# meyer-lab/cmtf-pls

Measured on AMD Instinct MI355X. Metric: nipals_iters_per_sec, higher is better.
Workload: dtype f32

## Files before the change

### cmtf_pls_amd/_lib.py

```python
from __future__ import annotations

import ctypes
import os
from ctypes import c_char_p, c_double, c_int, c_int64, c_size_t, c_uint32, c_uint64, c_void_p

_HERE = os.path.dirname(os.path.abspath(__file__))
LIB_PATH = os.environ.get("CMTFPLS_LIB") or os.path.join(_HERE, "lib", "libcmtfpls.so")

_P = c_void_p

class XcovBlock(ctypes.Structure):
    _fields_ = [("S", _P), ("S2", _P), ("colcnt", _P), ("n_samples", c_double), ("order", c_int), ("A", c_int), ("B", c_int),
                ("n_squarings", c_int), ("Z", _P), ("wA", _P), ("wB", _P), ("info", _P)]


class KfoldState(ctypes.Structure):
    _fields_ = [("I", c_int), ("A", c_int), ("B", c_int), ("M", c_int), ("K", c_int), ("R", c_int)] + [
        (name, _P) for name in ("fold_of", "S", "mean", "Yk", "Gy", "WA", "WB", "Q", "Wa", "Wb", "T", "Gt", "coef", "Rm", "tm",
                                "Tout", "vec", "n_iter", "status", "part")]


class CvCoupledBlock(ctypes.Structure):
    _fields_ = [("X", _P), ("order", c_int), ("A", c_int), ("B", c_int)]

# ... 23 lines not shown
    "cmtfpls_rank1_workspace_bytes": (c_size_t, [c_int, c_int]),
    "cmtfpls_rank1_score_f64": (c_int, [_P, c_int, c_int, _P, _P, _P, c_int, _P, c_int, _P, _P, c_size_t, _P]),
    "cmtfpls_rank1_f64": (c_int, [_P, c_int, c_int, _P, _P, _P, _P, c_int, _P, c_size_t, _P]),
    "cmtfpls_rank1_launches_f64": (c_int, [_P, c_int, c_int, _P, _P, _P, _P, c_int, _P, c_size_t, _P]),
    "cmtfpls_rank1_chain_enable": (None, [c_int]),
    "cmtfpls_rank1_chain_enabled": (c_int, []),
    "cmtfpls_normalize_f64": (c_int, [_P, c_int64, _P, _P]),
    "cmtfpls_rank1_tensor_workspace_bytes": (c_size_t, [_P, c_int]),
    "cmtfpls_rank1_tensor_f64": (c_int, [_P, _P, c_int, c_double, _P, c_int, _P, c_int, _P, c_size_t, _P]),
    "cmtfpls_kron_f64": (c_int, [_P, c_int, _P, c_int, _P, _P]),
    "cmtfpls_xcov_workspace_bytes": (c_size_t, [c_int64, c_int64, c_int]),
    "cmtfpls_xcov_f32": (c_int, [_P, c_int64, c_int64, _P, c_int, c_int, _P, c_int, _P, c_size_t, _P]),
    "cmtfpls_xcov_f64": (c_int, [_P, c_int64, c_int64, _P, c_int, c_int, _P, c_int, _P, c_size_t, _P]),
    "cmtfpls_quadform_f64": (c_int, [_P, c_int, _P, _P, _P, _P]),
    "cmtfpls_xcov_iterate_f64": (c_int, [_P, c_int, c_int, c_int, _P, _P, _P, _P, _P, c_int, _P, _P, _P, c_int, _P, c_size_t, _P, c_size_t, _P]),
    "cmtfpls_s_downdate_f64": (c_int, [_P, c_int, c_int, c_int, _P, _P, _P, _P, _P, _P]),
    "cmtfpls_project_rows_f32": (c_int, [_P, c_int64, c_int, c_int, c_int, _P, _P, _P, _P, c_int, _P]),
    "cmtfpls_project_rows_f64": (c_int, [_P, c_int64, c_int, c_int, c_int, _P, _P, _P, _P, c_int, _P]),
    "cmtfpls_project_rows2_f32": (c_int, [_P, c_int, c_int, _P, _P, _P, _P, c_int, c_int, _P, _P, _P, c_int64, c_int, _P, c_int, _P]),
    "cmtfpls_project_rows2_f64": (c_int, [_P, c_int, c_int, _P, _P, _P, _P, c_int, c_int, _P, _P, _P, c_int64, c_int, _P, c_int, _P]),
    "cmtfpls_project_rows_idx_f32": (c_int, [_P, _P, c_int64, c_int, c_int, c_int, _P, _P, _P, _P, c_int, _P]),
    "cmtfpls_project_rows_idx_f64": (c_int, [_P, _P, c_int64, c_int, c_int, c_int, _P, _P, _P, _P, c_int, _P]),
    "cmtfpls_project_rows2_idx_f32": (c_int, [_P, c_int, c_int, _P, _P, _P, _P, c_int, c_int, _P, _P, _P, _P, c_int64, c_int, _P, c_int, _P]),
    "cmtfpls_project_rows2_idx_f64": (c_int, [_P, c_int, c_int, _P, _P, _P, _P, c_int, c_int, _P, _P, _P, _P, c_int64, c_int, _P, c_int, _P]),
    "cmtfpls_allreduce_sum_f64": (c_int, [_P, _P, c_size_t, _P]),
    "cmtfpls_allreduce_sum_f32": (c_int, [_P, _P, c_size_t, _P]),
    "cmtfpls_axpy_scalar_f64": (c_int, [_P, c_int64, _P, _P, _P]),
    "cmtfpls_xcov_deflate_f32": (c_int, [_P, c_int64, c_int, c_int, _P, c_int, c_int, _P, _P, _P, _P, _P, _P, c_size_t, _P]),
    "cmtfpls_xcov_deflate_f64": (c_int, [_P, c_int64, c_int, c_int, _P, c_int, c_int, _P, _P, _P, _P, _P, _P, c_size_t, _P]),
    "cmtfpls_xcov_stats_workspace_bytes": (c_size_t, [c_int64, c_int64, c_int]),
# ... 170 lines not shown
```

### cmtf_pls_amd/backend.py

```python
from __future__ import annotations

import ctypes
from typing import Optional, Tuple

import torch

from . import _lib

_SUFFIX = {torch.float32: "f32", torch.float64: "f64"}


def _ptr(t: Optional[torch.Tensor]):
    return None if t is None else t.data_ptr()


def _int_pairs(pairs):
    flat = [int(v) for p in pairs for v in p]
    return (ctypes.c_int * len(flat))(*flat)


def chunk_size(n: int, per: int, budget: int, cap: Optional[int] = None) -> int:
    chunk = max(1, min(int(n), int(budget) // max(int(per), 1)))
    return chunk if cap is None else min(chunk, int(cap))

# ... 235 lines not shown
                          wB: torch.Tensor, status: torch.Tensor, q_new: torch.Tensor, G: torch.Tensor):
        M, P = S.shape
        wc = self._workspace("contract", self.lib.cmtfpls_mode0_contract_workspace_bytes(M, P))
        wr = self._workspace("rank1", self.lib.cmtfpls_rank1_workspace_bytes(A, B))
        keep = (S, q_cur, Z, wA, wB, status, q_new, G, wc, wr)
        fn = self.lib.cmtfpls_xcov_iterate_f64
        head = (_ptr(S), M, A, B, _ptr(q_cur), _ptr(Z), _ptr(wA), _ptr(wB), status[1:3].data_ptr())
        tail = (_ptr(wc), wc.numel(), _ptr(wr), wr.numel())
        qn, Gp, du2 = _ptr(q_new), _ptr(G), status[0:1].data_ptr()
        stream = self._stream

        def enqueue(n_squarings: int, first: bool, _keep=keep) -> None:
            rc = fn(*head, n_squarings, qn, Gp, du2, 1 if first else 0, *tail, stream())
            if rc:
                _lib.check(rc, "xcov_iterate")
        return enqueue

    def xcov_iterate(self, S: torch.Tensor, A: int, B: int, q_cur: torch.Tensor, Z: torch.Tensor, wA: torch.Tensor,
                     wB: torch.Tensor, info: torch.Tensor, n_squarings: int, q_new: torch.Tensor, G: torch.Tensor,
                     du2: torch.Tensor, first: bool) -> None:
        M, P = S.shape
        wc = self._workspace("contract", self.lib.cmtfpls_mode0_contract_workspace_bytes(M, P))
        wr = self._workspace("rank1", self.lib.cmtfpls_rank1_workspace_bytes(A, B))
        _lib.check(self.lib.cmtfpls_xcov_iterate_f64(_ptr(S), M, A, B, _ptr(q_cur), _ptr(Z), _ptr(wA), _ptr(wB), _ptr(info),
                                                     int(n_squarings), _ptr(q_new), _ptr(G), _ptr(du2), int(first),
                                                     _ptr(wc), wc.numel(), _ptr(wr), wr.numel(), self._stream()), "xcov_iterate")

    def xcov_blocks_plan(self, blocks, M: int, q_cur: torch.Tensor, tq: torch.Tensor, q_new: torch.Tensor, G: torch.Tensor,
                         status: torch.Tensor):
        nb = len(blocks)
# ... 785 lines not shown
```

### cmtf_pls_amd/csrc/rank1.hip

```cpp
#include "common.hpp"
#include <atomic>

namespace cmtfpls {

constexpr int kTile = 16;
constexpr int kMaxTiles = 256;
constexpr int kMaxSteps = 48;

struct Rank1Ctl {
  int done;
  int final_buf;
  int steps_used;
  int last_step;
  double pad[6];
};
__host__ __device__ __forceinline__ size_t rank1_ctl_bytes(int nt) {
  return sizeof(Rank1Ctl) + ((size_t)(kMaxSteps + 2) * nt + 2 * (size_t)nt * nt) * sizeof(double);
}
__device__ __forceinline__ double* ctl_trace(Rank1Ctl* c, int nt, int step) { return reinterpret_cast<double*>(c + 1) + (size_t)step * nt; }
__device__ __forceinline__ double* ctl_fro(Rank1Ctl* c, int nt, int which) {
  return reinterpret_cast<double*>(c + 1) + (size_t)(kMaxSteps + 2) * nt + (size_t)which * nt * nt;
}

__device__ __forceinline__ double pow2_scale_from_trace(const double* parts, int nt, double* tr_out) {
// ... 117 lines not shown
    if ((tid & 63) == 0) fsum[tid >> 6] = sq;
    __syncthreads();
    if (tid == 0) ctl_fro(ctl, nt, step & 1)[blockIdx.y * nt + blockIdx.x] = ((fsum[0] + fsum[1]) + fsum[2]) + fsum[3];
  }
  if (blockIdx.x == blockIdx.y) {
    if (tx == ty) diag[tx] = (i0 + ty < n) ? cacc : 0.0;
    __syncthreads();
    if (tid == 0) {
      double t = 0.0;
      for (int l = 0; l < kTile; ++l) t += diag[l];
      ctl_trace(ctl, nt, step)[blockIdx.x] = t;
    }
  }
}

constexpr unsigned long long kChainEmpty = ~0ull;
constexpr int kChainMaxSteps = 31;
constexpr int kChainSpin = 1 << 15;

__device__ __forceinline__ double chain_ld(const double* p) {
  return __longlong_as_double((long long)__hip_atomic_load(reinterpret_cast<const unsigned long long*>(p), __ATOMIC_RELAXED, __HIP_MEMORY_SCOPE_AGENT));
}
__device__ __forceinline__ void chain_st(double* p, double v) {
  unsigned long long b = (unsigned long long)__double_as_longlong(v);
  if (b == kChainEmpty) b = 0x7FF8000000000000ull;
  __hip_atomic_store(reinterpret_cast<unsigned long long*>(p), b, __ATOMIC_RELAXED, __HIP_MEMORY_SCOPE_AGENT);
}
__device__ __forceinline__ bool chain_empty(double v) { return (unsigned long long)__double_as_longlong(v) == kChainEmpty; }

__global__ __launch_bounds__(256) void chain_preset_kernel(unsigned long long* __restrict__ p, int64_t n) {
  for (int64_t i = (int64_t)blockIdx.x * 256 + threadIdx.x; i < n; i += (int64_t)gridDim.x * 256) p[i] = kChainEmpty;
}

#ifdef CMTFPLS_CHAIN_PROFILE
__device__ unsigned long long g_chain_prof[1024];
#define CHAIN_STAMP(slot) do { if (first_wg && tid == 0 && step < 32) g_chain_prof[step * 8 + (slot)] = __builtin_amdgcn_s_memrealtime(); } while (0)
#define CHAIN_COUNT(slot, v) do { if (first_wg && tid == 0 && step < 32) g_chain_prof[step * 8 + (slot)] = (unsigned long long)(v); } while (0)
#else
#define CHAIN_STAMP(slot) do { } while (0)
#define CHAIN_COUNT(slot, v) do { } while (0)
#endif

__global__ __launch_bounds__(kTile* kTile) void syrk_chain_kernel(const double* __restrict__ M0, int n, int k0,
                                                                 double* gbufs, double* trs, double* fros, double* gave_up,
                                                                 Rank1Ctl* __restrict__ ctl, int n_squarings) {
  constexpr int KC = 128, KW = 8, LDP = KC + 2;
// ... 368 lines not shown
  }
  for (; c < P; c += step) {
    const VT xv = ld_stream(reinterpret_cast<const VT*>(xr + c));
    double d = 0.0;
    d = fma(xv.e[0], sB[w.k], d);
    d = fma(xv.e[1], sB[w.k + 1], d);
    acc = fma(sA[w.j], d, acc);
    w.next();
  }
  acc = block_sum(acc, red[0]);
  if (threadIdx.x == 0) t[blockIdx.x] = acc;
}

static inline size_t align_up(size_t x, size_t a) { return (x + a - 1) / a * a; }

static std::atomic<int> g_chain_on{1};

static int chain_slots() {
  static int slots = 0;
  if (slots == 0) {
    int dev = 0, cus = 0;
    if (hipGetDevice(&dev) != hipSuccess || hipDeviceGetAttribute(&cus, hipDeviceAttributeMultiprocessorCount, dev) != hipSuccess || cus <= 0) cus = 256;
    slots = 2 * cus;
  }
  return slots;
}

}

using namespace cmtfpls;

extern "C" {

size_t cmtfpls_rank1_workspace_bytes(int A, int B) {
  if (A <= 0 || B <= 0) return 0;
  const size_t n = (size_t)(A < B ? A : B), k = (size_t)(A < B ? B : A);
  const size_t nt = (n + kTile - 1) / kTile;
  const size_t chain = nt * nt <= 256 ? align_up(((size_t)(kChainMaxSteps + 1) * (n * n + nt + nt * nt) + 1) * sizeof(double), 256) : 0;
  return align_up(rank1_ctl_bytes((int)nt), 256) + 3 * align_up(n * n * sizeof(double), 256) +
         align_up((size_t)A * B * sizeof(double), 256) + align_up(n * sizeof(double), 256) + align_up(k * sizeof(double), 256) + chain;
}

static int rank1_run(const double* Z, int A, int B, double* wA, double* wB, double* sigma, double* info,
                     int n_squarings, void* ws, size_t ws_bytes, void* stream, const double* S, int M, double* tq, bool allow_chain = true);

int cmtfpls_rank1_f64(const double* Z, int A, int B, double* wA, double* wB, double* sigma, double* info,
                      int n_squarings, void* ws, size_t ws_bytes, void* stream) {
  return rank1_run(Z, A, B, wA, wB, sigma, info, n_squarings, ws, ws_bytes, stream, nullptr, 0, nullptr);
}

#ifdef CMTFPLS_CHAIN_PROFILE
int cmtfpls_debug_chain_prof(unsigned long long* out) { return (int)hipMemcpyFromSymbol(out, HIP_SYMBOL(g_chain_prof), sizeof(unsigned long long) * 1024); }
#endif
void cmtfpls_rank1_chain_enable(int on) { g_chain_on.store((on == 1 || on == 2) ? on : 0, std::memory_order_relaxed); }
int cmtfpls_rank1_chain_enabled(void) { return g_chain_on.load(std::memory_order_relaxed); }

int cmtfpls_rank1_launches_f64(const double* Z, int A, int B, double* wA, double* wB, double* sigma, double* info,
                               int n_squarings, void* ws, size_t ws_bytes, void* stream) {
  return rank1_run(Z, A, B, wA, wB, sigma, info, n_squarings, ws, ws_bytes, stream, nullptr, 0, nullptr, false);
}

int cmtfpls_rank1_score_f64(const double* Z, int A, int B, double* wA, double* wB, double* info, int n_squarings,
                            const double* S, int M, double* tq, void* ws, size_t ws_bytes, void* stream) {
  if (!S || !tq || M <= 0) { set_error("rank1_score: bad argument"); return CMTFPLS_EINVAL; }
  const int64_t P = (int64_t)A * B;
  if (M > 64 || P < 8192 || (B % 2) != 0 || ((size_t)(((A + 1) & ~1) + B) * sizeof(double)) > 60 * 1024 ||
      (reinterpret_cast<uintptr_t>(S) & 15) != 0) {
    int rc = cmtfpls_rank1_f64(Z, A, B, wA, wB, nullptr, info, n_squarings, ws, ws_bytes, stream);
    if (rc == CMTFPLS_OK) rc = cmtfpls_score_s_f64(S, M, A, B, wA, wB, tq, stream);
    return rc;
  }
  return rank1_run(Z, A, B, wA, wB, nullptr, info, n_squarings, ws, ws_bytes, stream, S, M, tq);
}

static int rank1_run(const double* Z, int A, int B, double* wA, double* wB, double* sigma, double* info,
                     int n_squarings, void* ws, size_t ws_bytes, void* stream, const double* S, int M, double* tq, bool allow_chain) {
  if (!Z || !wA || !wB || A <= 0 || B <= 0) { set_error("rank1: bad argument"); return CMTFPLS_EINVAL; }
  const int n = A < B ? A : B, k = A < B ? B : A;
  if (n > kTile * kMaxTiles) { set_error("rank1: min(A, B) > 4096 unsupported"); return CMTFPLS_EUNSUPPORTED; }
  if ((size_t)n * sizeof(double) > 64 * 1024) { set_error("rank1: seed exceeds the LDS"); return CMTFPLS_EUNSUPPORTED; }
  if (n_squarings < 1) n_squarings = 1;
  if (n_squarings > kMaxSteps) n_squarings = kMaxSteps;
  if (!ws || ws_bytes < cmtfpls_rank1_workspace_bytes(A, B)) { set_error("rank1: workspace too small"); return CMTFPLS_EWORKSPACE; }
  hipStream_t st = (hipStream_t)stream;
  char* p = static_cast<char*>(ws);
  Rank1Ctl* ctl = reinterpret_cast<Rank1Ctl*>(p);
  p += align_up(rank1_ctl_bytes((n + kTile - 1) / kTile), 256);
  double* buf0 = reinterpret_cast<double*>(p);
  p += align_up((size_t)n * n * sizeof(double), 256);
  double* buf1 = reinterpret_cast<double*>(p);
  p += align_up((size_t)n * n * sizeof(double), 256);
// ... 13 lines not shown
    hipLaunchKernelGGL(transpose_kernel, dim3((unsigned)((tot + 255) / 256)), dim3(256), 0, st, Z, A, B, Zt);
    M0 = Zt;
  }
  const int nt = (n + kTile - 1) / kTile;
  const dim3 grid(nt, nt), block(kTile, kTile);
  const int ny_blocks = (k + 31) / 32;
  const double* gave = nullptr;
  if (allow_chain && g_chain_on.load(std::memory_order_relaxed) && nt * nt <= 256 && nt * nt <= chain_slots() && n_squarings <= kChainMaxSteps) {
    const size_t nn = (size_t)n * n, steps = (size_t)n_squarings + 1;
    double* gbufs = chain_region;
    double* trs = gbufs + steps * nn;
    double* fros = trs + steps * nt;
    double* gave_up = fros + steps * (size_t)nt * nt;
    gave = gave_up;
    const int64_t words = (int64_t)(steps * (nn + nt + (size_t)nt * nt) + 1);
    hipLaunchKernelGGL(chain_preset_kernel, dim3((unsigned)((words + 2047) / 2048)), dim3(256), 0, st, reinterpret_cast<unsigned long long*>(chain_region), words);
    const dim3 cgrid(nt, (g_chain_on.load(std::memory_order_relaxed) == 2 && nt > 1) ? nt - 1 : nt);
    hipLaunchKernelGGL(syrk_chain_kernel, cgrid, block, 0, st, M0, n, k, gbufs, trs, fros, gave_up, ctl, n_squarings);
    hipLaunchKernelGGL(rank1_seed_xy_kernel, dim3(ny_blocks + (n + 3) / 4), dim3(256), (size_t)n * sizeof(double), st,
                       M0, n, k, gbufs, (int64_t)nn, gbufs, ctl, n_squarings, ny_blocks, yv, xv);
  } else {
    hipLaunchKernelGGL(syrk_step_kernel, grid, block, 0, st, M0, n, k, k, buf0, ctl, 0, 0, g0keep);
    for (int s = 1; s <= n_squarings; ++s) {
      const double* in = (s & 1) ? buf0 : buf1;
      double* out = (s & 1) ? buf1 : buf0;
      hipLaunchKernelGGL(syrk_step_kernel, grid, block, 0, st, in, n, n, n, out, ctl, s, s & 1, (double*)nullptr);
    }
    hipLaunchKernelGGL(rank1_seed_xy_kernel, dim3(ny_blocks + (n + 3) / 4), dim3(256), (size_t)n * sizeof(double), st,
                       M0, n, k, buf0, (int64_t)(buf1 - buf0), g0keep, ctl, n_squarings & 1, ny_blocks, yv, xv);
  }
  if (S) {
// ... 11 lines not shown
```

### cmtf_pls_amd/csrc/small.hip

```cpp
#include "common.hpp"

namespace cmtfpls {

void launch_reduce_rows(const double* part, int nrows, int64_t P, double* out, hipStream_t st);

constexpr int kSmallBlocks = 128;
constexpr int kMaxGramDim = 64;
constexpr size_t kSmallWsBytes = (size_t)kSmallBlocks * kMaxGramDim * kMaxGramDim * sizeof(double);

__global__ __launch_bounds__(256) void gram_tn_kernel(const double* __restrict__ A, int lda, int a,
                                                     const double* __restrict__ B, int ldb, int b,
                                                     int64_t I, double* __restrict__ part, int TR) {
  extern __shared__ double lds[];
  double* As = lds;
  double* Bs = lds + TR * a;
  const int ab = a * b;
  const int64_t rows_per = (I + gridDim.x - 1) / gridDim.x;
  const int64_t r0 = (int64_t)blockIdx.x * rows_per;
  const int64_t r1 = (r0 + rows_per < I) ? r0 + rows_per : I;
  double acc[16];
#pragma unroll
  for (int s = 0; s < 16; ++s) acc[s] = 0.0;
  for (int64_t rb = r0; rb < r1; rb += TR) {
    const int nr = (int)((r1 - rb < TR) ? r1 - rb : TR);
// ... 152 lines not shown
    wB[c] = w;
  }
  __syncthreads();
  for (int m = wv; m < M; m += 16) {
    double acc = 0.0;
    for (int c = lane; c < P; c += 64) acc = fma(S2[(int64_t)m * P + c], wl[c], acc);
    acc = wave_sum(acc);
    if (lane == 0) tq[m] = acc;
  }
}

__global__ __launch_bounds__(1024) void q_update_kernel(const double* __restrict__ qpart, int nblk, int M,
                                                       double* __restrict__ q, int normalize,
                                                       const double* __restrict__ G, const double* __restrict__ q_prev,
                                                       double* __restrict__ du2) {
  __shared__ double part[64][17];
  __shared__ double qs[64];
  __shared__ double dq[64];
  __shared__ double red[16];
  const int tid = threadIdx.x, lane = tid & 63;
  const int Mp = (M <= 16) ? 16 : (M <= 32) ? 32 : 64;
  const int ngrp = 1024 / Mp;
  const int m = tid & (Mp - 1), grp = tid / Mp;
  double* pflat = &part[0][0];
  if (qpart) {
    double sacc = 0.0;
    const int msafe = (m < M) ? m : 0;
    for (int b0 = grp; b0 < nblk; b0 += 16 * ngrp) {
      double v[16];
#pragma unroll
      for (int k = 0; k < 16; ++k) {
        const int b = b0 + k * ngrp;
        v[k] = qpart[(int64_t)((b < nblk) ? b : nblk - 1) * M + msafe];
      }
#pragma unroll
      for (int k = 0; k < 16; ++k) sacc += (b0 + k * ngrp < nblk) ? v[k] : 0.0;
    }
    if (m >= M) sacc = 0.0;
    pflat[grp * (Mp + 1) + m] = sacc;
    __syncthreads();
    if (tid < M) {
      double tot = 0.0;
      for (int g = 0; g < ngrp; ++g) tot += pflat[g * (Mp + 1) + tid];
      qs[tid] = tot;
    }
  } else if (tid < M) {
    qs[tid] = q[tid];
  }
  __syncthreads();
  if (tid < 64) {
    double v = (lane < M) ? qs[lane] : 0.0;
    if (normalize) {
      const double nrm = sqrt(wave_sum(v * v));
      v = v / nrm;
    }
    if (lane < M) {
      q[lane] = v;
      if (G) dq[lane] = v - q_prev[lane];
    }
  }
  if (G) {
    __syncthreads();
    double sacc = 0.0;
    for (int idx = tid; idx < M * M; idx += 1024) {
      const int i = idx / M, j = idx - i * M;
      sacc = fma(dq[i] * G[idx], dq[j], sacc);
    }
    sacc = block_sum(sacc, red);
    if (tid == 0) du2[0] = sacc;
  }
}

__global__ __launch_bounds__(256) void s_downdate_kernel(double* __restrict__ S, int M, int64_t P, int B,
                                                        const double* __restrict__ ya, const double* __restrict__ wA,
                                                        const double* __restrict__ wB, const double* __restrict__ q,
                                                        const double* __restrict__ v) {
  const int64_t c = (int64_t)blockIdx.x * 256 + threadIdx.x;
  if (c >= P) return;
  const double w = wA[c / B] * wB[c % B];
  const double vc = v[c];
  for (int m = 0; m < M; ++m) {
    double sv = S[(int64_t)m * P + c];
    sv = fma(-ya[m], w, sv);
    sv = fma(-q[m], vc, sv);
    S[(int64_t)m * P + c] = sv;
  }
}

__global__ __launch_bounds__(256) void s_contract_kernel(const double* __restrict__ S, int M, int64_t P, const double* __restrict__ q,
                                                        double* __restrict__ Z) {
  const int64_t c = (int64_t)blockIdx.x * 256 + threadIdx.x;
  if (c >= P) return;
  double acc = 0.0;
#pragma unroll 8
  for (int m = 0; m < M; ++m) acc = fma(q[m], S[(int64_t)m * P + c], acc);
  Z[c] = acc;
}

__global__ __launch_bounds__(256) void axpy_scalar_kernel(double* __restrict__ y, int64_t n, const double* __restrict__ a,
                                                         const double* __restrict__ x) {
  const double av = a[0];
  for (int64_t i = (int64_t)blockIdx.x * 256 + threadIdx.x; i < n; i += (int64_t)gridDim.x * 256) y[i] = fma(-av, x ? x[i] : 1.0, y[i]);
}

__global__ __launch_bounds__(256) void kr_axpy_kernel(double* __restrict__ v, int64_t P, int B, const double* __restrict__ WA,
                                                     const double* __restrict__ WB, int ld, int k, const double* __restrict__ coef) {
  __shared__ double cs[64];
  for (int j = threadIdx.x; j < k; j += 256) cs[j] = coef[j];
  __syncthreads();
  const int64_t c = (int64_t)blockIdx.x * 256 + threadIdx.x;
  if (c >= P) return;
// ... 129 lines not shown
    set_error("xcov_iterate: bad argument");
    return CMTFPLS_EINVAL;
  }
  if (M > 64) { set_error("xcov_iterate: more than 64 responses"); return CMTFPLS_EUNSUPPORTED; }
  const int64_t P = (int64_t)A * B;
  int rc = CMTFPLS_OK;
  if (first) {
    hipLaunchKernelGGL(s_contract_kernel, dim3((unsigned)((P + 255) / 256)), dim3(256), 0, (hipStream_t)stream, S, M, P, q_cur, Z);
    rc = check_launch("xcov_iterate: s_contract");
  }
  if (rc == CMTFPLS_OK) rc = cmtfpls_rank1_score_f64(Z, A, B, wA, wB, info, n_squarings, S, M, q_new, ws_rank1, ws_rank1_bytes, stream);
  if (rc == CMTFPLS_OK) rc = cmtfpls_q_update_f64(nullptr, 0, M, q_new, 1, G, q_cur, du2, stream);
  return rc;
}

int cmtfpls_xcov_iterate_blocks_f64(const cmtfpls_xcov_block* blocks, int nb, int M, const double* q_cur, double* tq, double* q_new,
                                    const double* G, double* du2, int first, void* ws_rank1, size_t ws_rank1_bytes, void* stream) {
  if (!blocks || nb <= 0 || !q_cur || !tq || !q_new || !G || !du2 || M <= 0) { set_error("xcov_iterate_blocks: bad argument"); return CMTFPLS_EINVAL; }
  if (M > 64) { set_error("xcov_iterate_blocks: more than 64 responses"); return CMTFPLS_EUNSUPPORTED; }
  hipStream_t st = (hipStream_t)stream;
  int rc = CMTFPLS_OK;
  for (int b = 0; b < nb && rc == CMTFPLS_OK; ++b) {
    const cmtfpls_xcov_block& k = blocks[b];
    if (!k.S || !k.Z || !k.wA || !k.wB || k.A <= 0 || k.B <= 0 || (k.order != 2 && k.order != 3) || (k.order == 2 && k.A != 1) ||
        (k.order == 3 && !k.info)) {
      set_error("xcov_iterate_blocks: bad block");
      return CMTFPLS_EINVAL;
    }
    const int64_t P = (int64_t)k.A * k.B;
    if (k.order == 2 && P <= 8192) {
// ... 39 lines not shown
```

### cmtf_pls_amd/fitrun_xcov.py

```python
from __future__ import annotations

import math
from typing import Optional

import torch


class XcovMixin:
    def _iterate_xcov(self, it: int) -> Optional[float]:
        be = self.eng.be
        self._executed += 1

        blk0 = self.blocks[0]
        composite = (len(self.blocks) == 1 and len(blk0.shape) == 3 and not blk0.has_miss and self.M <= 64
                     and self.qn.data_ptr() == self.Tq.data_ptr() and hasattr(be, "xcov_iterate"))

        par = self._parity
        q_cur, q_new = self.qx[par], self.qx[par ^ 1]

        def seg(first: bool):
            if composite:
                be.xcov_iterate(self.S[0], blk0.A, blk0.B, q_cur, self.Zs[0], self.wA[0], self.wB[0], self.status[1:3],
                                self.sq_budget[0], q_new, self.Gy, self.status[0:1], first)
                return
# ... 47 lines not shown
        if pp is None:
            M = self.M
            second = {"Z": [], "wA": [], "wB": []}
            for b, blk in enumerate(self.blocks):
                second["Z"].append(be.empty(blk.A * blk.B))
                second["wA"].append(self.wA[b].clone())
                second["wB"].append(be.empty(blk.B))
            pp = self._pipe = {
                "q": [self.qx[0], self.qx[1], be.zeros(M)],
                "Z": [list(self.Zs), second["Z"]], "wA": [list(self.wA), second["wA"]], "wB": [list(self.wB), second["wB"]],
                "status": [be.zeros(1 + 2 * nb), be.zeros(1 + 2 * nb)],
                "plans": {}, "slots": {},
            }
            for st in pp["status"]:
                st[1::2] = 1.0
        plans = pp["plans"]

        def make_plan(it: int):
            s = it & 1
            st, q_cur, q_new = pp["status"][s], pp["q"][it % 3], pp["q"][(it + 1) % 3]
            if single:
                blk0 = self.blocks[0]
                if hasattr(be, "xcov_iterate_plan"):
                    one = be.xcov_iterate_plan(self.S[0], blk0.A, blk0.B, q_cur, pp["Z"][s][0], pp["wA"][s][0], pp["wB"][s][0], st,
                                               q_new, self.Gy)
                    return lambda nsq, first: one(nsq[0], first)
                return lambda nsq, first: be.xcov_iterate(self.S[0], blk0.A, blk0.B, q_cur, pp["Z"][s][0], pp["wA"][s][0],
                                                          pp["wB"][s][0], st[1:3], nsq[0], q_new, self.Gy, st[0:1], first)
            descr = [dict(S=self.S[b], S2=self.S2[b] if blk.has_miss else None, colcnt=blk.colcnt if blk.has_miss else None,
                          n_samples=self.n_total, order=len(blk.shape), A=blk.A, B=blk.B,
                          Z=pp["Z"][s][b], wA=pp["wA"][s][b], wB=pp["wB"][s][b]) for b, blk in enumerate(self.blocks)]
            return be.xcov_blocks_plan(descr, self.M, q_cur, self.Tq, q_new, self.Gy, st)

        def enqueue(it: int, first: bool = True):
            plan = plans.get(it % 6)
            if plan is None:
                plan = plans[it % 6] = make_plan(it)
            plan([n if it > 0 else min(self.sq_max, n + 4) for n in self.sq_budget], first)
            return be.status_snapshot(pp["status"][it & 1], it & 1, slots=pp["slots"])

        stats = self.pipeline_stats
        it, tok = 0, enqueue(0)
        du_prev = du = None
        while True:
            ahead = None
            if it + 1 < max_iter:
                predicted = None if (du is None or du_prev is None or du_prev <= 0.0) else du * (du / du_prev)
                if it == 0 or predicted is None or predicted >= tol:
                    ahead = enqueue(it + 1)
                    stats["ahead"] += 1
            host = be.status_wait(tok)
            short = [b for b in range(nb) if not host[1 + 2 * b] > 0.5 and self.sq_budget[b] < self.sq_max]
            if any(host[2 + 2 * b] < 0 for b in range(nb)):
# ... 174 lines not shown
```

### cmtf_pls_amd/options.py

```python
from __future__ import annotations

from dataclasses import dataclass, replace
from typing import Optional


@dataclass(frozen=True)
class EngineOptions:
    small_fit: bool = True
    small_fit_elements: int = 1 << 15
    xcov_nowrite: bool = True
    xcov_raw: bool = True
    xcov_raw_max_offset: float = 1e4
    project_raw_max_offset: float = 1e4
    xcov_one_read: bool = True
    xcov_pair_build: bool = True
    xcov_ssq_with_s: bool = True
    xcov_stats_with_s: bool = True
    xcov_deflate_build: bool = True
    xcov_pipeline: bool = True
    capture_collectives: bool = False
    project_split_rows: bool = True
    masked_folds: bool = False
    masked_folds_coupled: bool = False
    coupled_permutations: bool = False
    tensor_folds: bool = False
    tensor_folds_coupled: bool = False
    masked_tensor_folds: bool = False
    tensor_resamples_coupled: bool = False

    def but(self, **changes) -> "EngineOptions":
        return replace(self, **changes)


_DEFAULT_OPTIONS = EngineOptions()
# ... 11 lines not shown
```

### include/cmtfpls.h

```cpp
#ifndef CMTFPLS_H
#define CMTFPLS_H

#include <stddef.h>
#include <stdint.h>

#ifdef __cplusplus
extern "C" {
#endif

#define CMTFPLS_OK 0
#define CMTFPLS_EINVAL 1
#define CMTFPLS_EWORKSPACE 2
#define CMTFPLS_EHIP 3
#define CMTFPLS_EUNSUPPORTED 4

int cmtfpls_abi_version(void);
const char* cmtfpls_last_error(void);
int cmtfpls_clear_error(void);
int cmtfpls_status_to_host(const void* src, void* dst_host, size_t bytes, void* event, void* stream);

size_t cmtfpls_colstats_workspace_bytes(int64_t I, int64_t P);
int cmtfpls_colstats_f32(const float* X, int64_t I, int64_t P, double* colsum, double* colcnt,
                         void* ws, size_t ws_bytes, void* stream);
int cmtfpls_colstats_f64(const double* X, int64_t I, int64_t P, double* colsum, double* colcnt,
// ... 42 lines not shown
                             const double* wB, double* S, double* ssq, void* ws, size_t ws_bytes, void* stream);
size_t cmtfpls_xcov_ssq_workspace_bytes(int64_t I, int64_t P, int M);
size_t cmtfpls_xcov_stats_workspace_bytes(int64_t I, int64_t P, int M);
int cmtfpls_xcov_stats_f32(const float* X, int64_t I, int64_t P, const double* Y, int ldy, int M, double* S, double* stats,
                           void* ws, size_t ws_bytes, void* stream);
int cmtfpls_xcov_stats_f64(const double* X, int64_t I, int64_t P, const double* Y, int ldy, int M, double* S, double* stats,
                           void* ws, size_t ws_bytes, void* stream);
int cmtfpls_xcov_ssq_f32(const float* X, int64_t I, int64_t P, const double* Y, int ldy, int M, double* S, const double* mean,
                         double* ssq, void* ws, size_t ws_bytes, void* stream);
int cmtfpls_xcov_ssq_f64(const double* X, int64_t I, int64_t P, const double* Y, int ldy, int M, double* S, const double* mean,
                         double* ssq, void* ws, size_t ws_bytes, void* stream);
int cmtfpls_xcov_iterate_f64(const double* S, int M, int A, int B, const double* q_cur, double* Z, double* wA,
                             double* wB, double* info, int n_squarings, double* q_new, const double* G, double* du2,
                             int first, void* ws_contract, size_t ws_contract_bytes, void* ws_rank1,
                             size_t ws_rank1_bytes, void* stream);
typedef struct {
  const double* S;
  const double* S2;
  const double* colcnt;
  double n_samples;
  int order;
  int A, B;
  int n_squarings;
  double* Z;
  double* wA;
  double* wB;
  double* info;
} cmtfpls_xcov_block;
int cmtfpls_xcov_iterate_blocks_f64(const cmtfpls_xcov_block* blocks, int nb, int M, const double* q_cur, double* tq, double* q_new,
                                    const double* G, double* du2, int first, void* ws_rank1, size_t ws_rank1_bytes, void* stream);
// ... 298 lines not shown
```

Measured before the change: 766.8.

## Fuse NIPALS iteration tail: q update, next contraction and chain reset in one kernel

Splits the single-block xcov iteration into a head (S contraction) and a body. The body runs the fused rank-1 score without presetting the chain region, then launches one tail kernel that normalizes q, computes du2, contracts S with the new q to produce the next Z, and re-presets the dirty chain words for the next call. Launches per iteration drop from six to four. The cost is double-buffered Z, a persistent clean workspace, and correctness that depends on the chain region always being left clean between calls.

```diff
diff --git a/cmtf_pls_amd/_lib.py b/cmtf_pls_amd/_lib.py
--- a/cmtf_pls_amd/_lib.py
+++ b/cmtf_pls_amd/_lib.py
@@ -61,6 +61,9 @@
     "cmtfpls_xcov_f64": (c_int, [_P, c_int64, c_int64, _P, c_int, c_int, _P, c_int, _P, c_size_t, _P]),
     "cmtfpls_quadform_f64": (c_int, [_P, c_int, _P, _P, _P, _P]),
     "cmtfpls_xcov_iterate_f64": (c_int, [_P, c_int, c_int, c_int, _P, _P, _P, _P, _P, c_int, _P, _P, _P, c_int, _P, c_size_t, _P, c_size_t, _P]),
+    "cmtfpls_rank1_chain_clean_f64": (c_int, [c_int, c_int, _P, c_size_t, _P]),
+    "cmtfpls_xcov_iterate_head_f64": (c_int, [_P, c_int, c_int, c_int, _P, _P, _P]),
+    "cmtfpls_xcov_iterate_body_f64": (c_int, [_P, c_int, c_int, c_int, _P, _P, _P, _P, _P, _P, _P, _P, _P, _P, c_int, _P, c_size_t, _P]),
     "cmtfpls_s_downdate_f64": (c_int, [_P, c_int, c_int, c_int, _P, _P, _P, _P, _P, _P]),
     "cmtfpls_project_rows_f32": (c_int, [_P, c_int64, c_int, c_int, c_int, _P, _P, _P, _P, c_int, _P]),
     "cmtfpls_project_rows_f64": (c_int, [_P, c_int64, c_int, c_int, c_int, _P, _P, _P, _P, c_int, _P]),
diff --git a/cmtf_pls_amd/backend.py b/cmtf_pls_amd/backend.py
--- a/cmtf_pls_amd/backend.py
+++ b/cmtf_pls_amd/backend.py
@@ -273,6 +273,38 @@
             rc = fn(*head, n_squarings, qn, Gp, du2, 1 if first else 0, *tail, stream())
             if rc:
                 _lib.check(rc, "xcov_iterate")
+        return enqueue
+
+    def xcov_tail_workspace(self, S: torch.Tensor, A: int, B: int) -> Optional[torch.Tensor]:
+        M = S.shape[0]
+        rc = self.lib.cmtfpls_xcov_iterate_body_f64(_ptr(S), M, A, B, _ptr(S), _ptr(S) + 8, _ptr(S), _ptr(S), _ptr(S) + 8, _ptr(S),
+                                                    _ptr(S), _ptr(S), None, _ptr(S), 1, None, 0, self._stream())
+        if rc == 4:
+            return None
+        if rc != 2:
+            _lib.check(rc or 1, "xcov_iterate_body (probe)")
+        ws = torch.empty(max(int(self.lib.cmtfpls_rank1_workspace_bytes(A, B)), 256), dtype=torch.uint8, device=self.device)
+        _lib.check(self.lib.cmtfpls_rank1_chain_clean_f64(A, B, _ptr(ws), ws.numel(), self._stream()), "rank1_chain_clean")
+        return ws
+
+    def xcov_tail_plan(self, S: torch.Tensor, A: int, B: int, q_cur: torch.Tensor, Z: torch.Tensor, Z_next: torch.Tensor,
+                       wA: torch.Tensor, wB: torch.Tensor, status: torch.Tensor, tq: torch.Tensor, q_new: torch.Tensor,
+                       G: torch.Tensor, ws: torch.Tensor):
+        M, P = S.shape
+        keep = (S, q_cur, Z, Z_next, wA, wB, status, tq, q_new, G, ws)
+        head_fn, body_fn = self.lib.cmtfpls_xcov_iterate_head_f64, self.lib.cmtfpls_xcov_iterate_body_f64
+        head_args = (_ptr(S), M, A, B, _ptr(q_cur), _ptr(Z))
+        body_args = (_ptr(S), M, A, B, _ptr(Z), _ptr(Z_next), _ptr(q_cur), _ptr(tq), _ptr(q_new), _ptr(G), _ptr(wA), _ptr(wB),
+                     status[1:3].data_ptr(), status[0:1].data_ptr())
+        tail = (_ptr(ws), ws.numel())
+        stream = self._stream
+
+        def enqueue(n_squarings: int, head: bool, _keep=keep) -> None:
+            st = stream()
+            rc = head_fn(*head_args, st) if head else 0
+            rc = rc or body_fn(*body_args, n_squarings, *tail, st)
+            if rc:
+                _lib.check(rc, "xcov_iterate_body")
         return enqueue
 
     def xcov_iterate(self, S: torch.Tensor, A: int, B: int, q_cur: torch.Tensor, Z: torch.Tensor, wA: torch.Tensor,
diff --git a/cmtf_pls_amd/csrc/iter_bodies.hpp b/cmtf_pls_amd/csrc/iter_bodies.hpp
--- /dev/null
+++ b/cmtf_pls_amd/csrc/iter_bodies.hpp
@@ -0,0 +1,91 @@
+#pragma once
+
+#include "common.hpp"
+
+namespace cmtfpls {
+
+constexpr unsigned long long kChainEmpty = ~0ull;
+
+__device__ __forceinline__ void chain_preset_body(unsigned long long* __restrict__ p, int64_t n, int64_t first, int64_t stride) {
+  for (int64_t i = first; i < n; i += stride) p[i] = kChainEmpty;
+}
+
+__device__ __forceinline__ void s_contract_body(const double* __restrict__ S, int M, int64_t P, const double* q, double* __restrict__ Z,
+                                                int64_t c) {
+  if (c >= P) return;
+  double acc = 0.0;
+#pragma unroll 8
+  for (int m = 0; m < M; ++m) acc = fma(q[m], S[(int64_t)m * P + c], acc);
+  Z[c] = acc;
+}
+
+__device__ __forceinline__ double q_lane_body(const double* qs, int M, int lane, int normalize) {
+  double v = (lane < M) ? qs[lane] : 0.0;
+  if (normalize) {
+    const double nrm = sqrt(wave_sum(v * v));
+    v = v / nrm;
+  }
+  return v;
+}
+
+__device__ __forceinline__ void q_update_body(const double* __restrict__ qpart, int nblk, int M, const double* q_in, double* q_out,
+                                              int normalize, const double* __restrict__ G, const double* __restrict__ q_prev,
+                                              double* __restrict__ du2) {
+  __shared__ double part[64][17];
+  __shared__ double qs[64];
+  __shared__ double dq[64];
+  __shared__ double red[16];
+  const int tid = threadIdx.x, lane = tid & 63;
+  const int Mp = (M <= 16) ? 16 : (M <= 32) ? 32 : 64;
+  const int ngrp = 1024 / Mp;
+  const int m = tid & (Mp - 1), grp = tid / Mp;
+  double* pflat = &part[0][0];
+  if (qpart) {
+    double sacc = 0.0;
+    const int msafe = (m < M) ? m : 0;
+    for (int b0 = grp; b0 < nblk; b0 += 16 * ngrp) {
+      double v[16];
+#pragma unroll
+      for (int k = 0; k < 16; ++k) {
+        const int b = b0 + k * ngrp;
+        v[k] = qpart[(int64_t)((b < nblk) ? b : nblk - 1) * M + msafe];
+      }
+#pragma unroll
+      for (int k = 0; k < 16; ++k) sacc += (b0 + k * ngrp < nblk) ? v[k] : 0.0;
+    }
+    if (m >= M) sacc = 0.0;
+    pflat[grp * (Mp + 1) + m] = sacc;
+    __syncthreads();
+    if (tid < M) {
+      double tot = 0.0;
+      for (int g = 0; g < ngrp; ++g) tot += pflat[g * (Mp + 1) + tid];
+      qs[tid] = tot;
+    }
+  } else if (tid < M) {
+    qs[tid] = q_in[tid];
+  }
+  __syncthreads();
+  if (tid < 64) {
+    const double v = q_lane_body(qs, M, lane, normalize);
+    if (lane < M) {
+      q_out[lane] = v;
+      if (G) dq[lane] = v - q_prev[lane];
+    }
+  }
+  if (G) {
+    __syncthreads();
+    double sacc = 0.0;
+    for (int idx = tid; idx < M * M; idx += 1024) {
+      const int i = idx / M, j = idx - i * M;
+      sacc = fma(dq[i] * G[idx], dq[j], sacc);
+    }
+    sacc = block_sum(sacc, red);
+    if (tid == 0) du2[0] = sacc;
+  }
+}
+
+int rank1_score_clean(const double* Z, int A, int B, double* wA, double* wB, double* info, int n_squarings, const double* S, int M,
+                      double* tq, void* ws, size_t ws_bytes, void* stream, unsigned long long** dirty, int64_t* dirty_words);
+bool rank1_score_fused_shape(const double* S, int M, int A, int B);
+
+}
diff --git a/cmtf_pls_amd/csrc/rank1.hip b/cmtf_pls_amd/csrc/rank1.hip
--- a/cmtf_pls_amd/csrc/rank1.hip
+++ b/cmtf_pls_amd/csrc/rank1.hip
@@ -1,4 +1,5 @@
 #include "common.hpp"
+#include "iter_bodies.hpp"
 #include <atomic>
 
 namespace cmtfpls {
@@ -155,7 +156,6 @@
   }
 }
 
-constexpr unsigned long long kChainEmpty = ~0ull;
 constexpr int kChainMaxSteps = 31;
 constexpr int kChainSpin = 1 << 15;
 
@@ -170,7 +170,7 @@
 __device__ __forceinline__ bool chain_empty(double v) { return (unsigned long long)__double_as_longlong(v) == kChainEmpty; }
 
 __global__ __launch_bounds__(256) void chain_preset_kernel(unsigned long long* __restrict__ p, int64_t n) {
-  for (int64_t i = (int64_t)blockIdx.x * 256 + threadIdx.x; i < n; i += (int64_t)gridDim.x * 256) p[i] = kChainEmpty;
+  chain_preset_body(p, n, (int64_t)blockIdx.x * 256 + threadIdx.x, (int64_t)gridDim.x * 256);
 }
 
 #ifdef CMTFPLS_CHAIN_PROFILE
@@ -569,6 +569,11 @@
 
 static inline size_t align_up(size_t x, size_t a) { return (x + a - 1) / a * a; }
 
+static inline size_t chain_region_bytes(size_t n) {
+  const size_t nt = (n + kTile - 1) / kTile;
+  return nt * nt <= 256 ? align_up(((size_t)(kChainMaxSteps + 1) * (n * n + nt + nt * nt) + 1) * sizeof(double), 256) : 0;
+}
+
 static std::atomic<int> g_chain_on{1};
 
 static int chain_slots() {
@@ -585,19 +590,37 @@
 
 using namespace cmtfpls;
 
+static int rank1_run(const double* Z, int A, int B, double* wA, double* wB, double* sigma, double* info,
+                     int n_squarings, void* ws, size_t ws_bytes, void* stream, const double* S, int M, double* tq, bool allow_chain = true,
+                     bool clean_on_entry = false, unsigned long long** dirty = nullptr, int64_t* dirty_words = nullptr);
+
+namespace cmtfpls {
+
+bool rank1_score_fused_shape(const double* S, int M, int A, int B) {
+  const int64_t P = (int64_t)A * B;
+  return !(M > 64 || P < 8192 || (B % 2) != 0 || ((size_t)(((A + 1) & ~1) + B) * sizeof(double)) > 60 * 1024 ||
+           (reinterpret_cast<uintptr_t>(S) & 15) != 0);
+}
+
+int rank1_score_clean(const double* Z, int A, int B, double* wA, double* wB, double* info, int n_squarings, const double* S, int M,
+                      double* tq, void* ws, size_t ws_bytes, void* stream, unsigned long long** dirty, int64_t* dirty_words) {
+  *dirty = nullptr;
+  *dirty_words = 0;
+  return rank1_run(Z, A, B, wA, wB, nullptr, info, n_squarings, ws, ws_bytes, stream, S, M, tq, true, true, dirty, dirty_words);
+}
+
+}
+
 extern "C" {
 
 size_t cmtfpls_rank1_workspace_bytes(int A, int B) {
   if (A <= 0 || B <= 0) return 0;
   const size_t n = (size_t)(A < B ? A : B), k = (size_t)(A < B ? B : A);
   const size_t nt = (n + kTile - 1) / kTile;
-  const size_t chain = nt * nt <= 256 ? align_up(((size_t)(kChainMaxSteps + 1) * (n * n + nt + nt * nt) + 1) * sizeof(double), 256) : 0;
+  const size_t chain = chain_region_bytes(n);
   return align_up(rank1_ctl_bytes((int)nt), 256) + 3 * align_up(n * n * sizeof(double), 256) +
          align_up((size_t)A * B * sizeof(double), 256) + align_up(n * sizeof(double), 256) + align_up(k * sizeof(double), 256) + chain;
 }
-
-static int rank1_run(const double* Z, int A, int B, double* wA, double* wB, double* sigma, double* info,
-                     int n_squarings, void* ws, size_t ws_bytes, void* stream, const double* S, int M, double* tq, bool allow_chain = true);
 
 int cmtfpls_rank1_f64(const double* Z, int A, int B, double* wA, double* wB, double* sigma, double* info,
                       int n_squarings, void* ws, size_t ws_bytes, void* stream) {
@@ -615,12 +638,21 @@
   return rank1_run(Z, A, B, wA, wB, sigma, info, n_squarings, ws, ws_bytes, stream, nullptr, 0, nullptr, false);
 }
 
+int cmtfpls_rank1_chain_clean_f64(int A, int B, void* ws, size_t ws_bytes, void* stream) {
+  if (A <= 0 || B <= 0) { set_error("rank1_chain_clean: bad argument"); return CMTFPLS_EINVAL; }
+  const size_t total = cmtfpls_rank1_workspace_bytes(A, B), chain = chain_region_bytes((size_t)(A < B ? A : B));
+  if (!ws || ws_bytes < total) { set_error("rank1_chain_clean: workspace too small"); return CMTFPLS_EWORKSPACE; }
+  if (chain == 0) return CMTFPLS_OK;
+  const int64_t words = (int64_t)(chain / sizeof(double));
+  hipLaunchKernelGGL(chain_preset_kernel, dim3((unsigned)((words + 2047) / 2048)), dim3(256), 0, (hipStream_t)stream,
+                     reinterpret_cast<unsigned long long*>(static_cast<char*>(ws) + (total - chain)), words);
+  return check_launch("rank1_chain_clean");
+}
+
 int cmtfpls_rank1_score_f64(const double* Z, int A, int B, double* wA, double* wB, double* info, int n_squarings,
                             const double* S, int M, double* tq, void* ws, size_t ws_bytes, void* stream) {
   if (!S || !tq || M <= 0) { set_error("rank1_score: bad argument"); return CMTFPLS_EINVAL; }
-  const int64_t P = (int64_t)A * B;
-  if (M > 64 || P < 8192 || (B % 2) != 0 || ((size_t)(((A + 1) & ~1) + B) * sizeof(double)) > 60 * 1024 ||
-      (reinterpret_cast<uintptr_t>(S) & 15) != 0) {
+  if (!rank1_score_fused_shape(S, M, A, B)) {
     int rc = cmtfpls_rank1_f64(Z, A, B, wA, wB, nullptr, info, n_squarings, ws, ws_bytes, stream);
     if (rc == CMTFPLS_OK) rc = cmtfpls_score_s_f64(S, M, A, B, wA, wB, tq, stream);
     return rc;
@@ -629,7 +661,8 @@
 }
 
 static int rank1_run(const double* Z, int A, int B, double* wA, double* wB, double* sigma, double* info,
-                     int n_squarings, void* ws, size_t ws_bytes, void* stream, const double* S, int M, double* tq, bool allow_chain) {
+                     int n_squarings, void* ws, size_t ws_bytes, void* stream, const double* S, int M, double* tq, bool allow_chain,
+                     bool clean_on_entry, unsigned long long** dirty, int64_t* dirty_words) {
   if (!Z || !wA || !wB || A <= 0 || B <= 0) { set_error("rank1: bad argument"); return CMTFPLS_EINVAL; }
   const int n = A < B ? A : B, k = A < B ? B : A;
   if (n > kTile * kMaxTiles) { set_error("rank1: min(A, B) > 4096 unsupported"); return CMTFPLS_EUNSUPPORTED; }
@@ -673,7 +706,9 @@
     double* gave_up = fros + steps * (size_t)nt * nt;
     gave = gave_up;
     const int64_t words = (int64_t)(steps * (nn + nt + (size_t)nt * nt) + 1);
-    hipLaunchKernelGGL(chain_preset_kernel, dim3((unsigned)((words + 2047) / 2048)), dim3(256), 0, st, reinterpret_cast<unsigned long long*>(chain_region), words);
+    if (!clean_on_entry)
+      hipLaunchKernelGGL(chain_preset_kernel, dim3((unsigned)((words + 2047) / 2048)), dim3(256), 0, st, reinterpret_cast<unsigned long long*>(chain_region), words);
+    if (dirty) { *dirty = reinterpret_cast<unsigned long long*>(chain_region); *dirty_words = words; }
     const dim3 cgrid(nt, (g_chain_on.load(std::memory_order_relaxed) == 2 && nt > 1) ? nt - 1 : nt);
     hipLaunchKernelGGL(syrk_chain_kernel, cgrid, block, 0, st, M0, n, k, gbufs, trs, fros, gave_up, ctl, n_squarings);
     hipLaunchKernelGGL(rank1_seed_xy_kernel, dim3(ny_blocks + (n + 3) / 4), dim3(256), (size_t)n * sizeof(double), st,
diff --git a/cmtf_pls_amd/csrc/small.hip b/cmtf_pls_amd/csrc/small.hip
--- a/cmtf_pls_amd/csrc/small.hip
+++ b/cmtf_pls_amd/csrc/small.hip
@@ -1,4 +1,5 @@
 #include "common.hpp"
+#include "iter_bodies.hpp"
 
 namespace cmtfpls {
 
@@ -190,61 +191,7 @@
                                                        double* __restrict__ q, int normalize,
                                                        const double* __restrict__ G, const double* __restrict__ q_prev,
                                                        double* __restrict__ du2) {
-  __shared__ double part[64][17];
-  __shared__ double qs[64];
-  __shared__ double dq[64];
-  __shared__ double red[16];
-  const int tid = threadIdx.x, lane = tid & 63;
-  const int Mp = (M <= 16) ? 16 : (M <= 32) ? 32 : 64;
-  const int ngrp = 1024 / Mp;
-  const int m = tid & (Mp - 1), grp = tid / Mp;
-  double* pflat = &part[0][0];
-  if (qpart) {
-    double sacc = 0.0;
-    const int msafe = (m < M) ? m : 0;
-    for (int b0 = grp; b0 < nblk; b0 += 16 * ngrp) {
-      double v[16];
-#pragma unroll
-      for (int k = 0; k < 16; ++k) {
-        const int b = b0 + k * ngrp;
-        v[k] = qpart[(int64_t)((b < nblk) ? b : nblk - 1) * M + msafe];
-      }
-#pragma unroll
-      for (int k = 0; k < 16; ++k) sacc += (b0 + k * ngrp < nblk) ? v[k] : 0.0;
-    }
-    if (m >= M) sacc = 0.0;
-    pflat[grp * (Mp + 1) + m] = sacc;
-    __syncthreads();
-    if (tid < M) {
-      double tot = 0.0;
-      for (int g = 0; g < ngrp; ++g) tot += pflat[g * (Mp + 1) + tid];
-      qs[tid] = tot;
-    }
-  } else if (tid < M) {
-    qs[tid] = q[tid];
-  }
-  __syncthreads();
-  if (tid < 64) {
-    double v = (lane < M) ? qs[lane] : 0.0;
-    if (normalize) {
-      const double nrm = sqrt(wave_sum(v * v));
-      v = v / nrm;
-    }
-    if (lane < M) {
-      q[lane] = v;
-      if (G) dq[lane] = v - q_prev[lane];
-    }
-  }
-  if (G) {
-    __syncthreads();
-    double sacc = 0.0;
-    for (int idx = tid; idx < M * M; idx += 1024) {
-      const int i = idx / M, j = idx - i * M;
-      sacc = fma(dq[i] * G[idx], dq[j], sacc);
-    }
-    sacc = block_sum(sacc, red);
-    if (tid == 0) du2[0] = sacc;
-  }
+  q_update_body(qpart, nblk, M, q, q, normalize, G, q_prev, du2);
 }
 
 __global__ __launch_bounds__(256) void s_downdate_kernel(double* __restrict__ S, int M, int64_t P, int B,
@@ -265,12 +212,31 @@
 
 __global__ __launch_bounds__(256) void s_contract_kernel(const double* __restrict__ S, int M, int64_t P, const double* __restrict__ q,
                                                         double* __restrict__ Z) {
-  const int64_t c = (int64_t)blockIdx.x * 256 + threadIdx.x;
-  if (c >= P) return;
-  double acc = 0.0;
-#pragma unroll 8
-  for (int m = 0; m < M; ++m) acc = fma(q[m], S[(int64_t)m * P + c], acc);
-  Z[c] = acc;
+  s_contract_body(S, M, P, q, Z, (int64_t)blockIdx.x * 256 + threadIdx.x);
+}
+
+__global__ __launch_bounds__(1024) void xcov_tail_kernel(const double* tq, int M, double* __restrict__ q_new,
+                                                        const double* __restrict__ G, const double* __restrict__ q_cur,
+                                                        double* __restrict__ du2, const double* __restrict__ S, int64_t P,
+                                                        double* __restrict__ Z_next, int nc, unsigned long long* __restrict__ dirty,
+                                                        int64_t dirty_words) {
+  if (blockIdx.x == 0) {
+    q_update_body(nullptr, 0, M, tq, q_new, 1, G, q_cur, du2);
+    return;
+  }
+  if ((int)blockIdx.x <= nc) {
+    __shared__ double qs[64];
+    __shared__ double qn[64];
+    const int tid = threadIdx.x;
+    if (tid < M) qs[tid] = tq[tid];
+    __syncthreads();
+    if (tid < 64) qn[tid] = q_lane_body(qs, M, tid, 1);
+    __syncthreads();
+    s_contract_body(S, M, P, qn, Z_next, (int64_t)(blockIdx.x - 1) * 1024 + tid);
+    return;
+  }
+  const int64_t b = (int64_t)blockIdx.x - 1 - nc, nb = (int64_t)gridDim.x - 1 - nc;
+  chain_preset_body(dirty, dirty_words, b * 1024 + threadIdx.x, nb * 1024);
 }
 
 __global__ __launch_bounds__(256) void axpy_scalar_kernel(double* __restrict__ y, int64_t n, const double* __restrict__ a,
@@ -430,6 +396,37 @@
   return rc;
 }
 
+int cmtfpls_xcov_iterate_head_f64(const double* S, int M, int A, int B, const double* q, double* Z, void* stream) {
+  if (!S || !q || !Z || M <= 0 || A <= 0 || B <= 0) { set_error("xcov_iterate_head: bad argument"); return CMTFPLS_EINVAL; }
+  const int64_t P = (int64_t)A * B;
+  hipLaunchKernelGGL(s_contract_kernel, dim3((unsigned)((P + 255) / 256)), dim3(256), 0, (hipStream_t)stream, S, M, P, q, Z);
+  return check_launch("xcov_iterate_head");
+}
+
+int cmtfpls_xcov_iterate_body_f64(const double* S, int M, int A, int B, const double* Z, double* Z_next, const double* q_cur,
+                                  double* tq, double* q_new, const double* G, double* wA, double* wB, double* info, double* du2,
+                                  int n_squarings, void* ws_rank1, size_t ws_rank1_bytes, void* stream) {
+  if (!S || !Z || !Z_next || !q_cur || !tq || !q_new || !G || !wA || !wB || !du2 || M <= 0 || A <= 0 || B <= 0 || Z == Z_next ||
+      tq == q_new) {
+    set_error("xcov_iterate_body: bad argument");
+    return CMTFPLS_EINVAL;
+  }
+  if (!rank1_score_fused_shape(S, M, A, B)) {
+    set_error("xcov_iterate_body: outside the fused score (M <= 64, A * B >= 8192, B even, loadings within 60 KB, S 16-byte aligned)");
+    return CMTFPLS_EUNSUPPORTED;
+  }
+  unsigned long long* dirty = nullptr;
+  int64_t dirty_words = 0;
+  const int rc = rank1_score_clean(Z, A, B, wA, wB, info, n_squarings, S, M, tq, ws_rank1, ws_rank1_bytes, stream, &dirty, &dirty_words);
+  if (rc != CMTFPLS_OK) return rc;
+  const int64_t P = (int64_t)A * B;
+  const int nc = (int)((P + 1023) / 1024);
+  const int nclean = (int)((dirty_words + 8191) / 8192);
+  hipLaunchKernelGGL(xcov_tail_kernel, dim3((unsigned)(1 + nc + nclean)), dim3(1024), 0, (hipStream_t)stream, tq, M, q_new, G, q_cur, du2,
+                     S, P, Z_next, nc, dirty, dirty_words);
+  return check_launch("xcov_iterate_body: tail");
+}
+
 int cmtfpls_xcov_iterate_blocks_f64(const cmtfpls_xcov_block* blocks, int nb, int M, const double* q_cur, double* tq, double* q_new,
                                     const double* G, double* du2, int first, void* ws_rank1, size_t ws_rank1_bytes, void* stream) {
   if (!blocks || nb <= 0 || !q_cur || !tq || !q_new || !G || !du2 || M <= 0) { set_error("xcov_iterate_blocks: bad argument"); return CMTFPLS_EINVAL; }
diff --git a/cmtf_pls_amd/fitrun_xcov.py b/cmtf_pls_amd/fitrun_xcov.py
--- a/cmtf_pls_amd/fitrun_xcov.py
+++ b/cmtf_pls_amd/fitrun_xcov.py
@@ -85,13 +85,30 @@
             }
             for st in pp["status"]:
                 st[1::2] = 1.0
+            pp["tail"] = None
+            if single:
+                form = "six launches per iteration"
+                if self.eng.opt.xcov_tail and hasattr(be, "xcov_tail_plan"):
+                    blk0 = self.blocks[0]
+                    ws = be.xcov_tail_workspace(self.S[0], blk0.A, blk0.B)
+                    if ws is None:
+                        form += " (four declined: the shape is outside the fused score -- rows of >= 8192 elements, last mode even)"
+                    else:
+                        pp["tail"] = {"ws": ws, "tq": be.zeros(M)}
+                        form = "four launches per iteration (tail)"
+                self.pipeline_stats["form"] = form
         plans = pp["plans"]
+        tail = pp["tail"]
 
         def make_plan(it: int):
             s = it & 1
             st, q_cur, q_new = pp["status"][s], pp["q"][it % 3], pp["q"][(it + 1) % 3]
             if single:
                 blk0 = self.blocks[0]
+                if tail:
+                    four = be.xcov_tail_plan(self.S[0], blk0.A, blk0.B, q_cur, pp["Z"][s][0], pp["Z"][s ^ 1][0], pp["wA"][s][0],
+                                             pp["wB"][s][0], st, tail["tq"], q_new, self.Gy, tail["ws"])
+                    return lambda nsq, head: four(nsq[0], head)
                 if hasattr(be, "xcov_iterate_plan"):
                     one = be.xcov_iterate_plan(self.S[0], blk0.A, blk0.B, q_cur, pp["Z"][s][0], pp["wA"][s][0], pp["wB"][s][0], st,
                                                q_new, self.Gy)
@@ -107,7 +124,7 @@
             plan = plans.get(it % 6)
             if plan is None:
                 plan = plans[it % 6] = make_plan(it)
-            plan([n if it > 0 else min(self.sq_max, n + 4) for n in self.sq_budget], first)
+            plan([n if it > 0 else min(self.sq_max, n + 4) for n in self.sq_budget], (it == 0 or not first) if tail else first)
             return be.status_snapshot(pp["status"][it & 1], it & 1, slots=pp["slots"])
 
         stats = self.pipeline_stats
diff --git a/cmtf_pls_amd/options.py b/cmtf_pls_amd/options.py
--- a/cmtf_pls_amd/options.py
+++ b/cmtf_pls_amd/options.py
@@ -18,6 +18,7 @@
     xcov_stats_with_s: bool = True
     xcov_deflate_build: bool = True
     xcov_pipeline: bool = True
+    xcov_tail: bool = True
     capture_collectives: bool = False
     project_split_rows: bool = True
     masked_folds: bool = False
diff --git a/include/cmtfpls.h b/include/cmtfpls.h
--- a/include/cmtfpls.h
+++ b/include/cmtfpls.h
@@ -80,6 +80,11 @@
                              double* wB, double* info, int n_squarings, double* q_new, const double* G, double* du2,
                              int first, void* ws_contract, size_t ws_contract_bytes, void* ws_rank1,
                              size_t ws_rank1_bytes, void* stream);
+int cmtfpls_rank1_chain_clean_f64(int A, int B, void* ws, size_t ws_bytes, void* stream);
+int cmtfpls_xcov_iterate_head_f64(const double* S, int M, int A, int B, const double* q, double* Z, void* stream);
+int cmtfpls_xcov_iterate_body_f64(const double* S, int M, int A, int B, const double* Z, double* Z_next, const double* q_cur,
+                                  double* tq, double* q_new, const double* G, double* wA, double* wB, double* info, double* du2,
+                                  int n_squarings, void* ws_rank1, size_t ws_rank1_bytes, void* stream);
 typedef struct {
   const double* S;
   const double* S2;
```

Result: no change. 765.7 (-0.1%).
